# Rongjiehuang/FastDiff

Measured on AMD Instinct MI355X. Metric: real-time factor (audio-sec/wall-sec), N=4 reverse steps, 80x864 mel, higher is better.
Workload: dtype f32 results; 2-piece fp16 operands (22 bit) on fp16 MFMA, fp32 accumulate; GEMM as Winograd F(2,3); exact-fp32 twin; 1 GPU; BASELINE configs[1]: LJSpeech shape, batch=8 x 80x864 mel per GPU, N=4, HIP kernels + hipGraph sampler; batch_per_gpu=8, frames=864, reverse_steps=4, graph=True, weights=random init seed 1234 (no checkpoint offline), world_size=1, gpus_visible=1, oversubscribed=False

## Files before the change

fastdiff_amd/csrc/fd_api.cpp:

```cpp
#include <math.h>
#include <stddef.h>
#include <stdio.h>
#include <stdlib.h>
#include <string.h>

#include <algorithm>

#include "fd_kernels.h"
#include "fd_host.h"

std::string g_create_error;

static inline int gx_rows_host(int T) { return std::max(fdk_fast::gx_rows(T), fdk_fast::gw_pairs(T) * (fdk_fast::GW_ROWB / fdk_fast::GX_ROWB)); }

bool fd_prof_stamps(const fdk::Launch &L, const char *name, hipEvent_t *e0, hipEvent_t *e1)
{
    fd_context *c = L.ctx;
    if (c->profile != 1 || L.capturing) return false;
    hipEvent_t ev[2];
    for (int i = 0; i < 2; ++i) {
        if (!c->event_pool.empty()) { ev[i] = c->event_pool.back(); c->event_pool.pop_back(); }
        else if (hipEventCreate(&ev[i]) != hipSuccess) return false;
    }
    ProfEntry pe;
// ... 604 lines not shown
    h->pending.active = false;
    return resolve_call(h, p, mask);
}

static int sample_core(fd_handle h, const fd_context::SampleArgs &a, unsigned force_mask, long long ticket)
{
    int rc;
    const int B = a.B, T_io = a.T, T = bucket_frames(h, a.T), N = a.N;
    const int64_t L_io = (int64_t)T_io * fd::HOPT, Lp = (int64_t)T * fd::HOPT;
    hipStream_t stream = a.stream;
    Workspace &ws = h->ws;
    const size_t n_el = (size_t)B * T * fd::HOPT;
    const std::vector<unsigned long long> &ids = a.ids;
    constexpr int CHUNK = 8;
    StepMode mode = h->mode;
    const int np = hoist_mult(h, B, T, N);
    mode.hoist_np = np;
    mode.hoist_chunk = np > 1 && N > CHUNK;
    mode.fp32_mask = force_mask;
    mode.inline_fallback = force_mask != 0 || !h->host_fallback;
    std::vector<int> own_lens;
    const int *lens_eff = a.has_lens ? a.lens.data() : nullptr;
    if (!lens_eff && T != T_io) { own_lens.assign(B, T_io); lens_eff = own_lens.data(); }
    {
        fd_context::StageSlot *sl = nullptr;
        const size_t off_lens = sizeof(StepParams), off_ids = off_lens + ((sizeof(int) * B * np + 7) & ~(size_t)7);
        const size_t off_offs = off_ids + sizeof(unsigned long long) * B;
        const bool has_offs = !ids.empty() && !a.offs.empty();
        if ((rc = fd_stage_acquire(h, off_offs + sizeof(long long) * B, &sl)) != FD_OK) return rc;
        if ((rc = set_lens(h, lens_eff, B, T, stream, "fd_sample", reinterpret_cast<int *>(sl->host + off_lens), &mode.ragged, np)) != FD_OK)
            return rc;
        if (!ids.empty()) {
            memcpy(sl->host + off_ids, ids.data(), sizeof(unsigned long long) * B);
            FD_HIP(h, hipMemcpyAsync(ws.uid_dev, sl->host + off_ids, sizeof(unsigned long long) * B, hipMemcpyHostToDevice, stream));
        }
        if (has_offs) {
            memcpy(sl->host + off_offs, a.offs.data(), sizeof(long long) * B);
            FD_HIP(h, hipMemcpyAsync(ws.off_dev, sl->host + off_offs, sizeof(long long) * B, hipMemcpyHostToDevice, stream));
        }
        StepParams *p = reinterpret_cast<StepParams *>(sl->host);
        memcpy(p->table, a.table.data(), sizeof(fd_step) * N);
        p->z = a.z; p->seq = a.seq_out; p->seed = a.seed; p->n_steps = N; p->ddim = a.ddim ? 1 : 0; p->step_idx = 0; p->l4 = T * (fd::HOPT / 4);
        p->uids = ids.empty() ? nullptr : ws.uid_dev;
        p->offs4 = has_offs ? ws.off_dev : nullptr;
        p->l4_io = T_io * (fd::HOPT / 4); p->n4_io = (long long)B * p->l4_io;
        const size_t head = sizeof(fd_step) * N;
        FD_HIP(h, hipMemcpyAsync(ws.params, p, head, hipMemcpyHostToDevice, stream));
        const size_t off = offsetof(StepParams, z);
        FD_HIP(h, hipMemcpyAsync(reinterpret_cast<char *>(ws.params) + off, reinterpret_cast<const char *>(p) + off, sizeof(StepParams) - off,
                                 hipMemcpyHostToDevice, stream));
        if ((rc = fd_stage_commit(h, sl, stream)) != FD_OK) return rc;
    }
    fdk::Launch L = {h, stream, false, &mode};
    hipError_t e = fdk::copy_rows(L, ws.mel, T, a.mel, T_io, T_io, B * fd::COND);
    if (e == hipSuccess && a.x_T) e = fdk::copy_rows(L, ws.x, Lp, a.x_T, L_io, (int)L_io, B);
    if (e != hipSuccess) FD_FAIL(h, FD_ERR_HIP, "fd_sample: input copy failed: %s", hipGetErrorString(e));
    if (!a.x_T && (e = fdk::init_noise(L, ws.x, B, T * (fd::HOPT / 4), T_io * (fd::HOPT / 4), a.seed, ids.empty() ? nullptr : ws.uid_dev,
                                       ids.empty() || a.offs.empty() ? nullptr : ws.off_dev)) != hipSuccess)
        FD_FAIL(h, FD_ERR_HIP, "fd_sample: init_noise failed: %s", hipGetErrorString(e));
    if (a.seq_out && (e = fdk::copy_rows(L, a.seq_out, L_io, ws.x, Lp, (int)L_io, B)) != hipSuccess)
        FD_FAIL(h, FD_ERR_HIP, "fd_sample: sequence copy failed: %s", hipGetErrorString(e));
    auto copy_out = [&]() -> int {
        const hipError_t eo = fdk::copy_rows(L, a.out, L_io, ws.x, Lp, (int)L_io, B);
        if (eo != hipSuccess) FD_FAIL(h, FD_ERR_HIP, "fd_sample: output copy failed: %s", hipGetErrorString(eo));
        return FD_OK;
    };

    StepIO io = {ws.x, ws.mel, nullptr, nullptr, 1};
    {
        std::vector<float> ts(N);
        for (int k = 0; k < N; ++k) ts[k] = a.table[k].t;
        if (!(h->embed_cache && h->embed_valid && h->embed_B == B && h->embed_t == ts)) {
            h->embed_valid = false;
            if ((e = fdk::embed(L, io, B, N)) != hipSuccess) FD_FAIL(h, FD_ERR_HIP, "fd_sample: embed failed: %s", hipGetErrorString(e));
            h->embed_t.swap(ts);
            h->embed_B = B;
            h->embed_valid = true;
        }
    }
    if ((e = fdk::clear_range_flags(L)) != hipSuccess) FD_FAIL(h, FD_ERR_HIP, "fd_sample: %s", hipGetErrorString(e));

    if (np > 1) {
        const int64_t mel_n = (int64_t)B * fd::COND * T;
        if ((e = fdk::copy_rows(L, ws.mel_rep, T, ws.mel, T, T, B * fd::COND, np, mel_n)) != hipSuccess)
            FD_FAIL(h, FD_ERR_HIP, "fd_sample: mel replication failed: %s", hipGetErrorString(e));
    }
    if (np > 1 && !mode.hoist_chunk) {
        StepIO iop = {ws.x, ws.mel_rep, nullptr, nullptr, 0};
        e = fdk::kp_front(L, iop, B * N, T);
        if (e == hipSuccess) e = fdk::kp_gemm(L, B * N, T);
        if (e != hipSuccess) FD_FAIL(h, FD_ERR_HIP, "fd_sample: predictor launch failed: %s", hipGetErrorString(e));
    }
    if (force_mask != 0) {
        if ((rc = enqueue_steps(h, B, T, N, mode, stream)) != FD_OK) return rc;
        if ((rc = copy_out()) != FD_OK) return rc;
    } else if (h->host_fallback && N <= CHUNK) {
        if ((rc = enqueue_steps(h, B, T, N, mode, stream)) != FD_OK) return rc;
        const int slot = (int)(ticket & 1);
        FD_HIP(h, hipMemcpyAsync(h->flags_host + 32 * slot, ws.range_flag + 64, sizeof(int) * 32, hipMemcpyDeviceToHost, stream));
        FD_HIP(h, hipEventRecord(slot ? h->flags_done2 : h->flags_done, stream));
        if ((rc = copy_out()) != FD_OK) return rc;
        h->pending.active = true; h->pending.lazy = true; h->pending.slot = slot; h->pending.ticket = ticket;
        h->pending.B = B; h->pending.T = T; h->pending.T_io = T_io; h->pending.N = N; h->pending.first = 0; h->pending.count = N; h->pending.out = a.out;
        h->pending.stream = stream; h->pending.args = a;
    } else if (h->host_fallback) {
        FD_HIP(h, hipMemcpyAsync(ws.xsave, ws.x, sizeof(float) * n_el, hipMemcpyDeviceToDevice, stream));
        unsigned mask = 0;
        for (int first = 0; first < N; first += CHUNK) {
            const int count = std::min(CHUNK, N - first);
            const bool last = first + count == N;
            ++h->n_pieces;
            if (mask != 0) ++h->n_pieces_fp32;
            if (first > 0 && mask == 0) FD_HIP(h, hipMemcpyAsync(ws.xsave, ws.x, sizeof(float) * n_el, hipMemcpyDeviceToDevice, stream));
            mode.fp32_mask = mask;
            mode.inline_fallback = mask != 0;
            if ((rc = enqueue_steps(h, B, T, count, mode, stream)) != FD_OK) return rc;
            if (mask != 0) continue;
            FD_HIP(h, hipMemcpyAsync(h->flags_host, ws.range_flag + 64, sizeof(int) * 32, hipMemcpyDeviceToHost, stream));
            FD_HIP(h, hipEventRecord(h->flags_done, stream));
            h->pending.active = true; h->pending.lazy = false; h->pending.slot = 0; h->pending.ticket = ticket;
            h->pending.B = B; h->pending.T = T; h->pending.T_io = T_io; h->pending.N = N; h->pending.first = first; h->pending.count = count; h->pending.out = a.out;
            h->pending.stream = stream; h->pending.mode = mode;
            if (last) break;
            int redone = resolve_pending(h, &mask);
            if (redone < 0) return redone;
        }
        if ((rc = copy_out()) != FD_OK) return rc;
    } else {
        if ((rc = enqueue_steps(h, B, T, N, mode, stream)) != FD_OK) return rc;
        if ((rc = copy_out()) != FD_OK) return rc;
    }
    h->last_B = B; h->last_T = T;
    return fd_mark_tail(h, stream);
}

int fd_sample(fd_handle h, const float *mel, int B, int T, const int *lens, const fd_step *table, int N, int ddim,
              const float *x_T, const float *z, uint64_t seed, float *out, float *seq_out, void *stream_)
{
    std::vector<unsigned long long> ids;
    std::vector<long long> offs;
    if (h) { ids.swap(h->noise_ids); offs.swap(h->noise_offs); }
    int rc = check_common(h, B, T, "fd_sample");
    if (rc != FD_OK) return rc;
    if ((rc = fd_follow_stream(h, (hipStream_t)stream_)) != FD_OK) return rc;
    if (h->gen) {
        if (!mel || !table || !out) FD_FAIL(h, FD_ERR_INVALID, "fd_sample: null pointer");
        if (N <= 0 || N > 1024) FD_FAIL(h, FD_ERR_INVALID, "fd_sample: N=%d outside 1..1024", N);
        if (!ids.empty() && (int)ids.size() != B) FD_FAIL(h, FD_ERR_INVALID, "fd_sample: fd_set_noise_streams gave %d stream ids but B=%d", (int)ids.size(), B);
        for (int b = 0; lens && b < B; ++b)
            if (lens[b] < 1 || lens[b] > T) FD_FAIL(h, FD_ERR_INVALID, "fd_sample: lens[%d] = %d outside [1, T=%d]", b, lens[b], T);
        if ((rc = fdg::sample(h, mel, B, T, lens, table, N, ddim, x_T, z, seed, ids, out, seq_out, (hipStream_t)stream_)) != FD_OK) return rc;
        ++h->ticket_counter;
        h->last_B = B; h->last_T = T;
        return fd_mark_tail(h, (hipStream_t)stream_);
    }
    const bool lazy = h->host_fallback && N >= 1 && N <= 8;
    const int Tp = bucket_frames(h, T);
    if ((rc = check_common(h, B, Tp, "fd_sample")) != FD_OK) return rc;
    const int np = (N >= 1 && N <= 1024) ? hoist_mult(h, B, Tp, N) : 1;
    const bool ws_ok = workspace_fits(h, B, Tp, np);
    fd_context::PendingCall prev;
    if (lazy && ws_ok && h->pending.active && h->pending.lazy) {
        prev = h->pending;
        h->pending.active = false;
    } else if ((rc = fd_settle(h)) != FD_OK) return rc;
    auto finish_prev = [&]() -> int {
        if (!prev.active) return FD_OK;
        unsigned mask = 0;
        const fd_context::PendingCall cur = h->pending;
        h->pending.active = false;
        const int r = resolve_call(h, prev, &mask);
        h->pending = cur;
        prev.active = false;
        return r < 0 ? r : FD_OK;
    };
    if (!mel || !table || !out) { finish_prev(); FD_FAIL(h, FD_ERR_INVALID, "fd_sample: null pointer"); }
    if (N <= 0 || N > 1024) { finish_prev(); FD_FAIL(h, FD_ERR_INVALID, "fd_sample: N=%d outside 1..1024", N); }
    if (!ids.empty() && (int)ids.size() != B) {
        finish_prev();
        FD_FAIL(h, FD_ERR_INVALID, "fd_sample: fd_set_noise_streams gave %d stream ids but B=%d", (int)ids.size(), B);
    }
    if (!offs.empty() && offs.size() != ids.size()) { finish_prev(); FD_FAIL(h, FD_ERR_INVALID, "fd_sample: noise offsets without their stream ids"); }
    for (int b = 0; lens && b < B; ++b)
        if (lens[b] < 1 || lens[b] > T) {
            finish_prev();
            FD_FAIL(h, FD_ERR_INVALID, "fd_sample: lens[%d] = %d outside [1, T=%d]", b, lens[b], T);
        }
    if ((rc = ensure_workspace(h, B, Tp, np)) != FD_OK) { finish_prev(); return rc; }
    fd_context::SampleArgs a;
    a.mel = mel; a.B = B; a.T = T; a.N = N; a.ddim = ddim;
    a.has_lens = lens != nullptr;
    if (lens) a.lens.assign(lens, lens + B);
    a.table.assign(table, table + N);
    a.x_T = x_T; a.z = z; a.seed = seed; a.out = out; a.seq_out = seq_out; a.stream = (hipStream_t)stream_;
    a.ids.swap(ids);
    a.offs.swap(offs);
    const long long ticket = ++h->ticket_counter;
    h->n_pieces = h->n_pieces_redone = h->n_pieces_fp32 = 0;
    h->call_fp32_mask = 0;
    rc = sample_core(h, a, 0u, ticket);
    const int rc_prev = finish_prev();
    h->last_B = B; h->last_T = Tp;
    if (rc != FD_OK || rc_prev != FD_OK) return rc != FD_OK ? rc : rc_prev;
    if (!h->defer_check) return fd_settle(h);
    return FD_OK;
}

int64_t fd_sample_ticket(fd_handle h) { return h ? (int64_t)h->ticket_counter : FD_ERR_INVALID; }

static int ticket_redone(fd_handle h, long long ticket)
{
    for (long long t : h->redone_ring)
        if (t == ticket && t != 0) return 1;
    return 0;
}

int fd_sample_settle(fd_handle h, int64_t ticket)
{
    if (!h) return FD_ERR_INVALID;
    if (ticket <= 0 || ticket > h->ticket_counter) FD_FAIL(h, FD_ERR_INVALID, "fd_sample_settle: unknown ticket %lld", (long long)ticket);
    if (h->pending.active && h->pending.ticket <= ticket) {
        FD_HIP(h, hipSetDevice(h->device));
        unsigned mask = 0;
        const int r = resolve_pending(h, &mask);
        if (r < 0) return r;
    }
    return ticket_redone(h, ticket);
}

int fd_sample_check(fd_handle h)
{
    if (!h) return FD_ERR_INVALID;
    if (!h->pending.active) return 0;
    FD_HIP(h, hipSetDevice(h->device));
    unsigned mask = 0;
    return resolve_pending(h, &mask);
}

int fd_set_noise_streams(fd_handle h, const uint64_t *stream_ids, int B)
{
    if (!h || B < 0 || (B > 0 && !stream_ids)) return FD_ERR_INVALID;
    h->noise_ids.assign(stream_ids, stream_ids + B);
    h->noise_offs.clear();
    return FD_OK;
}

int fd_set_option(fd_handle h, const char *key, const char *value)
{
    if (!h || !key || !value) return FD_ERR_INVALID;
    {
        const int rcs = fd_settle(h);
        if (rcs != FD_OK) return rcs;
    }
    const std::string k(key), v(value);
    static const char *stage_names[ST_COUNT] = {"embed", "first", "dblock", "kp_front", "kp_gemm", "convt", "lvc", "final"};
    auto parse_mode = [&](bool &dst) -> int {
        if (v == "fast") dst = true;
        else if (v == "naive") dst = false;
        else FD_FAIL(h, FD_ERR_INVALID, "fd_set_option: %s expects fast|naive, got '%s'", key, value);
        return FD_OK;
    };
    if (k == "kernels") {
        bool m = true;
        int rc = parse_mode(m);
        if (rc != FD_OK) return rc;
        for (int i = 0; i < ST_COUNT; ++i) h->mode.fast[i] = m;
        return FD_OK;
    }
    if (k.compare(0, 8, "kernels.") == 0) {
        for (int i = 0; i < ST_COUNT; ++i)
            if (k.substr(8) == stage_names[i]) return parse_mode(h->mode.fast[i]);
        FD_FAIL(h, FD_ERR_INVALID, "fd_set_option: unknown stage '%s'", key);
    }
    static const struct { const char *key, *a, *b; void (*set)(fd_context *, bool); } choices[] = {
        {"gemm", "f16x2", "fp32", [](fd_context *c, bool a) { c->mode.gemm_f16 = a; }},
        {"gemm_form", "winograd", "direct", [](fd_context *c, bool a) { c->mode.gemm_wino = a; }},
        {"lvc", "f16x2", "fp32", [](fd_context *c, bool a) { c->mode.lvc_f16 = a; }},
        {"conv", "f16x2", "fp32", [](fd_context *c, bool a) { c->mode.conv_f16 = a; }},
        {"lvc_h8", "mfma", "valu", [](fd_context *c, bool a) { c->mode.lvc_h8_mfma = a; }},
        {"fallback", "graph", "host", [](fd_context *c, bool a) { c->host_fallback = !a; }},
        {"lvc_dx", "gather", "copy", [](fd_context *c, bool a) { c->lvc_dx_gather = a; }},
        {"mel", "pwg", "tacotron", [](fd_context *c, bool a) { c->mel_variant = a ? MEL_PWG : MEL_TACOTRON; }},
    };
    for (const auto &ch : choices) {
        if (k != ch.key) continue;
        if (v != ch.a && v != ch.b) FD_FAIL(h, FD_ERR_INVALID, "fd_set_option: %s expects %s|%s, got '%s'", key, ch.a, ch.b, value);
        ch.set(h, v == ch.a);
        return FD_OK;
    }
    const bool on = (v == "1" || v == "true" || v == "on");
    if (k == "fuse_final") { h->mode.fuse_final = on; return FD_OK; }
    if (k == "fuse_up") { h->mode.fuse_up = on; return FD_OK; }
    if (k == "fuse_advance") { h->mode.fuse_advance = on; return FD_OK; }
    if (k == "embed_cache") { h->embed_cache = on; return FD_OK; }
    if (k == "hoist") {
        if (v == "auto") h->hoist_mode = 1;
        else if (v == "on") h->hoist_mode = 2;
        else if (v == "off") h->hoist_mode = 0;
        else FD_FAIL(h, FD_ERR_INVALID, "fd_set_option: hoist expects auto|on|off, got '%s'", value);
        return FD_OK;
    }
    if (k == "graph") { h->use_graph = on; return FD_OK; }
    if (k == "defer_check") { h->defer_check = on; return FD_OK; }
    if (k == "t_bucket" || k == "graph_cache") {
        char *end = nullptr;
        const long n = strtol(value, &end, 10);
        if (end == value || *end != 0 || n < 0 || n > 65536 || (k == "graph_cache" && n < 1))
            FD_FAIL(h, FD_ERR_INVALID, "fd_set_option: %s expects an integer (t_bucket: frames, 0 = exact T; graph_cache: graphs kept, >= 1), got '%s'", key, value);
        if (k == "t_bucket") h->t_bucket = (int)n;
        else h->max_graphs = (int)n;
        return FD_OK;
    }
    if (k == "profile") { h->profile = (v == "events") ? 2 : (on ? 1 : 0); return FD_OK; }
    if (k == "taps") { h->mode.keep_taps = on; return FD_OK; }
    FD_FAIL(h, FD_ERR_INVALID, "fd_set_option: unknown option '%s'", key);
}

}
```

fastdiff_amd/csrc/fd_internal.h:

```cpp
#pragma once
#include <hip/hip_runtime.h>
#include <hip/hip_ext.h>
#include <stdint.h>
#include <string.h>
#include <map>
#include <string>
#include <vector>

#include "../../include/fastdiff_hip.h"
#include "../../include/fastdiff_hip_ext.h"
#include "../../include/fastdiff_hip_train.h"

namespace fd {
constexpr int C = 32;
constexpr int COND = 80;
constexpr int HID = 64;
constexpr int NBLK = 3;
constexpr int LAYERS = 4;
constexpr int HOPT = 256;
constexpr int E_IN = 128, E_MID = 512, E_OUT = 512;
constexpr int KLAYER = 2 * C * C * 3;
constexpr int KW = KLAYER * LAYERS;
constexpr int KB = 2 * C * LAYERS;
constexpr int KREC = KW + KB;
__host__ __device__ constexpr int ratio(int n) { return n == 2 ? 4 : 8; }
__host__ __device__ constexpr int hop(int n) { return n == 0 ? 8 : (n == 1 ? 64 : 256); }
__host__ __device__ constexpr int down_factor(int d) { return d == 0 ? 4 : 8; }

__host__ __device__ inline int kernel_row(int out) { return (out & 15) + 16 * (out >> 5); }
__host__ __device__ inline int kernel_tile(int out) { return (out & 31) >> 4; }
__host__ __device__ inline int kernel_index(int layer, int in, int out, int tap)
{
    const int kk = tap * C + in, kg = kk >> 4, g = (kk >> 3) & 1, e = kk & 7;
    const int mt = kernel_tile(out), lane = kernel_row(out) + 32 * g;
    return layer * KLAYER + ((mt * 6 + kg) * 64 + lane) * 8 + e;
}
__host__ __device__ inline int bias_index(int layer, int out) { return KW + layer * 64 + kernel_tile(out) * 32 + kernel_row(out); }
}

struct ConvW {
    const float *w = nullptr;
    const float *b = nullptr;
};

struct DevWeights {
    ConvW first, final_;
    struct { ConvW res, conv[3]; } down[fd::NBLK];
    struct { ConvW fc_t, up, kp_in, kp_res[6], kc, bc, convs[fd::LAYERS]; } blk[fd::NBLK];
    const float *fc_t1_T = nullptr, *fc_t1_b = nullptr, *fc_t2_T = nullptr, *fc_t2_b = nullptr;
    const float *fc_t_T[fd::NBLK] = {}, *fc_t_b[fd::NBLK] = {};
    const float *embed_table = nullptr;
    const float *down_pack[fd::NBLK][4] = {};
    const uint16_t *down_h2[fd::NBLK][4] = {};
    bool dblock_f16_ok = false;
    const float *lvc_conv_pack[fd::NBLK][fd::LAYERS] = {};
    const uint16_t *lvc_conv_h2[fd::NBLK][fd::LAYERS] = {};
    const uint16_t *lvc_conv_h16[fd::LAYERS] = {};
    bool lvc_f16_ok = false;
    const float *kp_in_pack[fd::NBLK] = {};
    const float *kp_res_pack[fd::NBLK][6] = {};
    const uint16_t *kp_in_h2[fd::NBLK] = {};
    const uint16_t *kp_res_h2[fd::NBLK][6] = {};
    bool kpf_f16_ok = false;
    const float *gemm_pack[fd::NBLK] = {};
    const float *gemm_bias[fd::NBLK] = {};
    const uint16_t *gemm_h2_pack[fd::NBLK] = {};
    bool gemm_f16_ok = false;
    const uint16_t *gemm_w_pack[fd::NBLK] = {};
    bool gemm_w_ok = false;
    const float *up_pack[fd::NBLK] = {};
    const uint16_t *up_h2[fd::NBLK] = {};
    bool convt_f16_ok = false;
    const float *final_fuse = nullptr;
    const int *kc_perm = nullptr;
    const int *bc_perm = nullptr;
};

struct StepParams {
    fd_step table[1024];
    const float *z;
    float *seq;
    unsigned long long seed;
    int n_steps;
    int ddim;
    int step_idx;
    int l4;
    const unsigned long long *uids;
    int l4_io;
    long long n4_io;
    const long long *offs4;
};

enum Stage { ST_EMBED = 0, ST_FIRST, ST_DBLOCK, ST_KP_FRONT, ST_KP_GEMM, ST_CONVT, ST_LVC, ST_FINAL, ST_COUNT };

struct StepMode {
    bool fast[ST_COUNT] = {true, true, true, true, true, true, true, true};
    bool gemm_f16 = true;
    bool gemm_wino = true;
    bool lvc_f16 = true;
    bool conv_f16 = true;
    bool lvc_h8_mfma = true;
    bool fuse_final = true;
    bool fuse_up = true;
    bool fuse_advance = true;
    bool keep_taps = false;
    unsigned fp32_mask = 0;
    bool inline_fallback = true;
    bool ragged = false;
    int hoist_np = 1;
    bool hoist_chunk = false;

    bool operator==(const StepMode &o) const
    {
        for (int i = 0; i < ST_COUNT; ++i)
            if (fast[i] != o.fast[i]) return false;
        return gemm_f16 == o.gemm_f16 && gemm_wino == o.gemm_wino && lvc_f16 == o.lvc_f16 && conv_f16 == o.conv_f16 &&
               lvc_h8_mfma == o.lvc_h8_mfma && fuse_final == o.fuse_final && fuse_up == o.fuse_up && fuse_advance == o.fuse_advance &&
               keep_taps == o.keep_taps && fp32_mask == o.fp32_mask && inline_fallback == o.inline_fallback && ragged == o.ragged &&
               hoist_np == o.hoist_np && hoist_chunk == o.hoist_chunk;
    }
};

struct Workspace {
    int B = 0;
    int64_t frames = 0;
    int64_t rows = 0;
    float *noise = nullptr;
    float *embed_h2 = nullptr;
    float *a[4] = {};
    float *kp_h0 = nullptr, *kp_hA = nullptr, *kp_hB = nullptr;
    float *kpack = nullptr;
    float *h_f16 = nullptr;
    int *lens_dev = nullptr;
    unsigned long long *uid_dev = nullptr;
    long long *off_dev = nullptr;
    float *xsave = nullptr;
    int *range_flag = nullptr;
    float *xA = nullptr, *xB = nullptr;
    float *xtap[fd::NBLK] = {};
    int64_t pframes = 0, prows = 0, plens = 0;
    float *mel_rep = nullptr;
    float *mel = nullptr;
    float *x = nullptr;
    float *eps_acc = nullptr;
    float *steps = nullptr;
    StepParams *params = nullptr;
    size_t bytes = 0;
};

struct ProfEntry { std::string name; hipEvent_t e0, e1; };
struct Scratch { float *p = nullptr; size_t bytes = 0; };

struct MelTables {
    const float *tab = nullptr;
    const int *fb_lo = nullptr, *fb_n = nullptr, *fb_off = nullptr;
    const float *fb_w = nullptr;
};
enum MelVariant { MEL_PWG = 0, MEL_TACOTRON = 1, MEL_VARIANTS = 2 };

struct FoldedParam { std::vector<float> w, b; };
struct WeightImage {
    std::vector<char> bytes;
    std::vector<std::pair<const void **, size_t>> fields;
    template <class T> void add(const T *&dst, const std::vector<T> &v)
    {
        const size_t off = (bytes.size() + 255) & ~(size_t)255;
        bytes.resize(off + v.size() * sizeof(T));
        memcpy(bytes.data() + off, v.data(), v.size() * sizeof(T));
        fields.push_back({reinterpret_cast<const void **>(&dst), off});
    }
};
namespace fdg {
struct Net;
int validate(const fd_config &c, std::string &why);
int create(fd_context *c);
void destroy(fd_context *c);
int hop_total(const fd_context *c);
int pack_weights(fd_context *c, const std::map<std::string, FoldedParam> &f, WeightImage &img);
int forward(fd_context *c, const float *x, const float *mel, const float *steps, int B, int T, const int *lens, float *eps_out, hipStream_t stream);
int sample(fd_context *c, const float *mel, int B, int T, const int *lens, const fd_step *table, int N, int ddim, const float *x_T, const float *z,
           unsigned long long seed, const std::vector<unsigned long long> &ids, float *out, float *seq_out, hipStream_t stream);
}

struct fd_context {
    fd_config cfg;
    fdg::Net *gen = nullptr;
    int device = 0;
    int num_cus = 256;
    std::string err;
    bool committed = false;
    StepMode mode;
    bool use_graph = true;
    int profile = 0;
    std::vector<unsigned long long> noise_ids;
    std::vector<long long> noise_offs;
    bool host_fallback = true;
    std::map<std::string, std::pair<std::vector<int64_t>, std::vector<float>>> raw;
    void *weight_arena = nullptr;
    DevWeights w;
    Workspace ws;
    bool lvc_dx_gather = true;
    std::vector<float> embed_t;
    int embed_B = 0;
    bool embed_valid = false;
    bool embed_cache = true;
    MelTables mel[MEL_VARIANTS];
    int mel_variant = MEL_PWG;
    std::vector<float> mel_bank[MEL_VARIANTS];
    bool mel_bank_user[MEL_VARIANTS] = {false, false};
    std::vector<void *> mel_allocs;
    int last_B = 0, last_T = 0;
    hipStream_t cap_stream = nullptr;
    hipStream_t last_stream = nullptr;
    bool have_last_stream = false;
    hipEvent_t ev_switch = nullptr;
    bool tail_marked = false;
    int hoist_mode = 1;
    struct StepGraph { int B, T, steps; StepMode mode; hipGraph_t graph; hipGraphExec_t exec; unsigned long long last_use; };
    std::vector<StepGraph> graphs;
    unsigned long long graph_clock = 0;
    struct RetiredGraph { hipGraph_t graph; hipGraphExec_t exec; hipEvent_t done; };
    std::vector<RetiredGraph> retired;
    int max_graphs = 64;
    int t_bucket = 32;
    long long n_graph_captures = 0, n_graph_hits = 0, n_graph_evictions = 0;
    bool defer_check = false;
    static constexpr int STAGE_SLOTS = 8;
    struct StageSlot { char *host = nullptr; size_t cap = 0; hipEvent_t done = nullptr; };
    StageSlot stage[STAGE_SLOTS];
    unsigned stage_next = 0;
    struct SampleArgs {
        const float *mel = nullptr;
        int B = 0, T = 0, N = 0, ddim = 0;
        bool has_lens = false;
        std::vector<int> lens;
        std::vector<fd_step> table;
        const float *x_T = nullptr, *z = nullptr;
        unsigned long long seed = 0;
        float *out = nullptr, *seq_out = nullptr;
        hipStream_t stream = nullptr;
        std::vector<unsigned long long> ids;
        std::vector<long long> offs;
    };
    struct PendingCall {
        bool active = false;
        bool lazy = false;
        int slot = 0;
        long long ticket = 0;
        int B = 0, T = 0, N = 0, first = 0, count = 0;
        int T_io = 0;
        float *out = nullptr;
        hipStream_t stream = nullptr;
        StepMode mode;
        SampleArgs args;
    } pending;
    long long ticket_counter = 0;
    long long n_pieces = 0, n_pieces_redone = 0, n_pieces_fp32 = 0, n_calls_redone = 0;
    unsigned call_fp32_mask = 0;
    long long redone_ring[16] = {};
    unsigned redone_next = 0;
    int *flags_host = nullptr;
    hipEvent_t flags_done = nullptr, flags_done2 = nullptr;
    void *scratch = nullptr;
    Scratch lvc_scratch;
    Scratch kconv_scratch;
    Scratch cconv_scratch;
    Scratch span_scratch;
    Scratch step_scratch;
    std::vector<ProfEntry> prof_pending;
    std::vector<hipEvent_t> event_pool;
    std::map<std::string, std::pair<int64_t, double>> prof_acc;
};

enum Pipe { PIPE_F16_THEN_F32, PIPE_F16_ONLY, PIPE_F32_ONLY };
inline Pipe fd_pipe(const StepMode &m, bool f16_possible, int flag_word)
{
    if (!f16_possible || ((m.fp32_mask >> flag_word) & 1u)) return PIPE_F32_ONLY;
    return m.inline_fallback ? PIPE_F16_THEN_F32 : PIPE_F16_ONLY;
}
inline bool front_writes_h_image(const StepMode &m, const DevWeights &w)
{
    return m.fast[ST_KP_FRONT] && fd_pipe(m, m.conv_f16 && w.kpf_f16_ok, 19) != PIPE_F32_ONLY &&
           fd_pipe(m, m.gemm_f16 && w.gemm_f16_ok, 0) != PIPE_F32_ONLY && !(m.gemm_wino && w.gemm_w_ok);
}
inline bool last_lvc_fuses_final(const StepMode &m, const DevWeights &w)
{
    return m.fast[ST_LVC] && m.fast[ST_FINAL] && !m.keep_taps && m.fuse_final &&
           fd_pipe(m, m.lvc_f16 && w.lvc_f16_ok, 1 + 2 * fd::LAYERS + 3) != PIPE_F32_ONLY;
}

struct StepIO {
    const float *x_in;
    const float *mel;
    const float *steps;
    float *eps_out;
    int sampler;
    int hoist_step = 0;
    bool advance = false;
};

namespace fdk {
struct Launch {
    fd_context *ctx;
    hipStream_t stream;
    bool capturing;
    const StepMode *mode = nullptr;
};
hipError_t embed(const Launch &L, const StepIO &io, int B, int n_steps);
hipError_t first_conv(const Launch &L, const StepIO &io, int B, int T);
hipError_t dblock(const Launch &L, const StepIO &io, int d, int B, int T);
hipError_t kp_front(const Launch &L, const StepIO &io, int B, int T);
hipError_t kp_gemm(const Launch &L, int B, int T);
hipError_t advance_step(const Launch &L);
hipError_t clear_range_flags(const Launch &L, int set_step = 0);
hipError_t mel_frontend(const Launch &L, const float *wav, int B, int64_t n_samples, float *mel, int T);
hipError_t init_noise(const Launch &L, float *x, int B, int l4, int l4_io, unsigned long long seed, const unsigned long long *uids,
                      const long long *offs4 = nullptr);
constexpr int SPAN_MAX_WINDOWS = 8;
struct SpanWindows {
    int n;
    long long start[SPAN_MAX_WINDOWS];
    int len[SPAN_MAX_WINDOWS];
    long long c0[SPAN_MAX_WINDOWS];
    int clen[SPAN_MAX_WINDOWS];
};
hipError_t span_gather(const Launch &L, const SpanWindows &w, int Wp, const float *mel, const float *x_T, const float *z, int nz,
                       long long mel_first, long long mel_frames, float *mel_w, float *x_w, float *z_w);
hipError_t span_scatter(const Launch &L, const SpanWindows &w, int Wp, const float *x_w, long long t0, float *out);
hipError_t copy_rows(const Launch &L, float *dst, int64_t dpitch, const float *src, int64_t spitch, int width, int rows, int reps = 1,
                     int64_t rep_stride = 0);
hipError_t peak_normalize_int16(const Launch &L, const float *wav, int B, int64_t len, int16_t *pcm, const long long *valid_dev);
}

bool fd_prof_stamps(const fdk::Launch &L, const char *name, hipEvent_t *e0, hipEvent_t *e1);
void fd_prof_begin(const fdk::Launch &L, const char *name);
void fd_prof_end(const fdk::Launch &L);

#define FD_LAUNCH(L, name, kernel, grid, block, shmem, ...)                                  \
    do {                                                                                     \
        hipEvent_t ev0__ = nullptr, ev1__ = nullptr;                                         \
        if (fd_prof_stamps(L, name, &ev0__, &ev1__)) {                                       \
            hipExtLaunchKernelGGL(kernel, grid, block, shmem, (L).stream, ev0__, ev1__, 0, __VA_ARGS__); \
        } else {                                                                             \
            fd_prof_begin(L, name);                                                          \
            hipLaunchKernelGGL(kernel, grid, block, shmem, (L).stream, __VA_ARGS__);         \
            fd_prof_end(L);                                                                  \
        }                                                                                    \
        hipError_t e__ = hipGetLastError();                                                  \
        if (e__ != hipSuccess) return e__;                                                   \
    } while (0)
```

fastdiff_amd/csrc/fd_kernels_dblock.hip:

```cpp
#include "fd_kernels_common.h"

namespace fdk_fast {

constexpr int DB_LD = 136;
constexpr int DB_STRIDE = 114;

template <int DIL, bool LRELU>
__device__ __forceinline__ void conv96_tile(f32x16 &acc, const float4 (&wa)[12], const float *in, int ld, int col, int hi)
{
    const int o[3] = {opaque(hi * ld + col - DIL), opaque(hi * ld + col), opaque(hi * ld + col + DIL)};
#pragma unroll
    for (int s = 0; s < 48; ++s) {
        const int tap = s >> 4, c2 = (2 * s) & 31;
        float v = in[o[tap] + c2 * ld];
        if (LRELU) v = lrelu(v, 0.2f);
        acc = mfma32(f4c(wa[s >> 2], s & 3), v, acc);
    }
}

template <int F>
__global__ void __launch_bounds__(256, 2) k_dblock(const float *__restrict__ xin, float *__restrict__ out,
                                                   const float *__restrict__ p0, const float *__restrict__ p1,
                                                   const float *__restrict__ p2, const float *__restrict__ pr,
                                                   const float *__restrict__ b0, const float *__restrict__ b1,
                                                   const float *__restrict__ b2, const float *__restrict__ br, int Lin, int Lo,
                                                   const int *__restrict__ run_if, const int *__restrict__ lens, int per_frame)
{
    __shared__ __attribute__((aligned(16))) float xs[fd::C * DB_LD];
    if (run_if && *run_if == 0) return;
    __shared__ __attribute__((aligned(16))) float hA[fd::C * DB_LD];
    __shared__ __attribute__((aligned(16))) float hB[fd::C * DB_LD];
    const int b = blockIdx.y, tid = threadIdx.x, lane = tid & 63, wave = tid >> 6, l31 = lane & 31, hi = lane >> 5;
    const int pbase = blockIdx.x * DB_STRIDE - 7;
    const int Lob = lens ? lens[b] * per_frame : Lo;
    if (blockIdx.x * DB_STRIDE >= Lob) return;
    {
        constexpr int NK = fd::C * DB_LD / 256;
        float v[NK];
#pragma unroll
        for (int k = 0; k < NK; ++k) {
            const int idx = k * 256 + tid, ci = idx / DB_LD, cc = idx - ci * DB_LD, p = pbase + cc - 4;
            v[k] = (cc >= 4 && cc < 132 && p >= 0 && p < Lob) ? xin[((int64_t)b * fd::C + ci) * Lin + (int64_t)p * F] : 0.0f;
        }
#pragma unroll
        for (int k = 0; k < NK; ++k) {
            const int idx = k * 256 + tid;
            xs[idx] = v[k];
            hA[idx] = 0.0f;
            hB[idx] = 0.0f;
        }
    }
    __syncthreads();
    const int c = wave * 32 + l31;
    const int p = pbase + c;
    const bool inside = (p >= 0 && p < Lob);
    float4 wa[12];
    f32x16 acc;
#pragma unroll
    for (int i = 0; i < 12; ++i) wa[i] = reinterpret_cast<const float4 *>(p0)[i * 64 + lane];
#pragma unroll
    for (int r = 0; r < 16; ++r) acc[r] = b0[drow(r, hi)];
    conv96_tile<1, true>(acc, wa, xs, DB_LD, 4 + c, hi);
#pragma unroll
    for (int r = 0; r < 16; ++r) hA[drow(r, hi) * DB_LD + 4 + c] = inside ? acc[r] : 0.0f;
    __syncthreads();
#pragma unroll
    for (int i = 0; i < 12; ++i) wa[i] = reinterpret_cast<const float4 *>(p1)[i * 64 + lane];
#pragma unroll
    for (int r = 0; r < 16; ++r) acc[r] = b1[drow(r, hi)];
    conv96_tile<2, true>(acc, wa, hA, DB_LD, 4 + c, hi);
#pragma unroll
    for (int r = 0; r < 16; ++r) hB[drow(r, hi) * DB_LD + 4 + c] = inside ? acc[r] : 0.0f;
    __syncthreads();
#pragma unroll
    for (int i = 0; i < 12; ++i) wa[i] = reinterpret_cast<const float4 *>(p2)[i * 64 + lane];
#pragma unroll
    for (int r = 0; r < 16; ++r) acc[r] = b2[drow(r, hi)] + br[drow(r, hi)];
    conv96_tile<4, true>(acc, wa, hB, DB_LD, 4 + c, hi);
    {
        float4 wr[4];
#pragma unroll
        for (int i = 0; i < 4; ++i) wr[i] = reinterpret_cast<const float4 *>(pr)[i * 64 + lane];
#pragma unroll
        for (int s = 0; s < 16; ++s) acc = mfma32(f4c(wr[s >> 2], s & 3), xs[(2 * s + hi) * DB_LD + 4 + c], acc);
    }
    if (inside && c >= 7 && c < 7 + DB_STRIDE) {
#pragma unroll
        for (int r = 0; r < 16; ++r) out[((int64_t)b * fd::C + drow(r, hi)) * Lo + p] = acc[r];
    }
}

constexpr int DBH_ROWS = 136;

template <int DIL>
__device__ __forceinline__ void conv96_h2(f32x16 &ah, f32x16 &al, const float4 (&wa)[2][6], const char *img, int c, int hi)
{
    int off[3][2][2];
#pragma unroll
    for (int tap = 0; tap < 3; ++tap)
#pragma unroll
        for (int p = 0; p < 2; ++p)
#pragma unroll
            for (int c2 = 0; c2 < 2; ++c2) off[tap][p][c2] = h2_off(4 + c + (tap - 1) * DIL, p * 4 + c2 * 2 + hi);
#pragma unroll
    for (int kg = 0; kg < 6; ++kg) {
        const float4 b1 = *reinterpret_cast<const float4 *>(img + off[kg >> 1][0][kg & 1]);
        const float4 b2 = *reinterpret_cast<const float4 *>(img + off[kg >> 1][1][kg & 1]);
        ah = mfma_f16(wa[0][kg], b1, ah);
        al = mfma_f16(wa[0][kg], b2, al);
        al = mfma_f16(wa[1][kg], b1, al);
    }
}
__device__ __forceinline__ void store_act_h2(char *img, const f32x16 &ah, const f32x16 &al, int c, int hi, bool inside, float &mx)
{
    const int row = 4 + c;
#pragma unroll
    for (int j = 0; j < 4; ++j) {
        float v[4];
#pragma unroll
        for (int i = 0; i < 4; ++i) {
            v[i] = inside ? lrelu(fmaf(al[4 * j + i], GX_INV_SCALE, ah[4 * j + i]), 0.2f) : 0.0f;
            mx = fmaxf(mx, fabsf(v[i]));
        }
        uint2 ph, pl;
        split2(v[0], v[1], ph.x, pl.x);
        split2(v[2], v[3], ph.y, pl.y);
        *reinterpret_cast<uint2 *>(img + h2_off(row, j) + 8 * hi) = ph;
        *reinterpret_cast<uint2 *>(img + h2_off(row, 4 + j) + 8 * hi) = pl;
    }
}

#ifndef FD_DBLOCK_OCC
#define FD_DBLOCK_OCC 3
#endif
template <int F, bool AUDIO>
__global__ void __launch_bounds__(256, FD_DBLOCK_OCC) k_dblock_h2(const float *__restrict__ xin, float *__restrict__ out,
                                                      const float4 *__restrict__ p0, const float4 *__restrict__ p1,
                                                      const float4 *__restrict__ p2, const float4 *__restrict__ pr,
                                                      const float *__restrict__ b0, const float *__restrict__ b1,
                                                      const float *__restrict__ b2, const float *__restrict__ br, int Lin, int Lo,
                                                      int *__restrict__ range_flag, const int *__restrict__ lens, int per_frame,
                                                      const float *__restrict__ audio, const float *__restrict__ fw,
                                                      const float *__restrict__ fb)
{
    __shared__ __attribute__((aligned(16))) char xl[DBH_ROWS * 128];
    __shared__ __attribute__((aligned(16))) char xr[DBH_ROWS * 128];
    __shared__ __attribute__((aligned(16))) char ha[DBH_ROWS * 128];
    const int b = blockIdx.y, tid = threadIdx.x, lane = tid & 63, wave = tid >> 6, l31 = lane & 31, hi = lane >> 5;
    const int pbase = blockIdx.x * DB_STRIDE - 7;
    const int Lob = lens ? lens[b] * per_frame : Lo;
    if (blockIdx.x * DB_STRIDE >= Lob || skip_after_previous_overflow(range_flag)) return;
    float mx = 0.0f;
    __shared__ float fwl[AUDIO ? 256 : 1];
    if constexpr (AUDIO) {
        fwl[tid] = tid < 224 ? fw[tid] : fb[tid - 224];
        __syncthreads();
    }
    {
        float v[2][8];
#pragma unroll
        for (int k = 0; k < 2; ++k) {
            const int u = k * 256 + tid, cg = u >> 7, cc = u & 127, p = pbase + cc;
            const bool ok = p >= 0 && p < Lob;
            if (AUDIO) {
                const int Lb = Lob * F, t = p * F;
                const float *xa = audio + (int64_t)b * Lin;
                float xv[7];
#pragma unroll
                for (int i = 0; i < 7; ++i) xv[i] = (ok && t - 3 + i >= 0 && t - 3 + i < Lb) ? xa[t - 3 + i] : 0.0f;
                const int o0 = __builtin_amdgcn_readfirstlane(cg) * 8;
#pragma unroll
                for (int c = 0; c < 8; ++c) {
                    float r = fwl[224 + o0 + c];
#pragma unroll
                    for (int i = 0; i < 7; ++i) r += fwl[(o0 + c) * 7 + i] * xv[i];
                    v[k][c] = ok ? r : 0.0f;
                }
            } else {
#pragma unroll
                for (int c = 0; c < 8; ++c) v[k][c] = ok ? xin[((int64_t)b * fd::C + cg * 8 + c) * Lin + (int64_t)p * F] : 0.0f;
            }
        }
        if (tid < 128) {
            const int g = tid >> 4, row = g < 4 ? g : 128 + g, part = tid & 15;
            *reinterpret_cast<uint2 *>(xl + row * 128 + part * 8) = make_uint2(0u, 0u);
            *reinterpret_cast<uint2 *>(xr + row * 128 + part * 8) = make_uint2(0u, 0u);
            *reinterpret_cast<uint2 *>(ha + row * 128 + part * 8) = make_uint2(0u, 0u);
        }
#pragma unroll
        for (int k = 0; k < 2; ++k) {
            const int u = k * 256 + tid, cg = u >> 7, cc = u & 127;
            float a[8];
#pragma unroll
            for (int c = 0; c < 8; ++c) { mx = fmaxf(mx, fabsf(v[k][c])); a[c] = lrelu(v[k][c], 0.2f); }
            float4 ph, pl;
            split8(v[k], ph, pl);
            *reinterpret_cast<float4 *>(xr + h2_off(4 + cc, cg)) = ph;
            *reinterpret_cast<float4 *>(xr + h2_off(4 + cc, 4 + cg)) = pl;
            split8(a, ph, pl);
            *reinterpret_cast<float4 *>(xl + h2_off(4 + cc, cg)) = ph;
            *reinterpret_cast<float4 *>(xl + h2_off(4 + cc, 4 + cg)) = pl;
        }
    }
    __syncthreads();
    const int c = wave * 32 + l31;
    const int p = pbase + c;
    const bool inside = (p >= 0 && p < Lob);
    float4 wa[2][6];
    f32x16 ah, al;
    auto load_w = [&](const float4 *pk) {
#pragma unroll
        for (int q = 0; q < 2; ++q)
#pragma unroll
            for (int kg = 0; kg < 6; ++kg) wa[q][kg] = pk[(q * 6 + kg) * 64 + lane];
    };
    load_w(p0);
#pragma unroll
    for (int r = 0; r < 16; ++r) { ah[r] = b0[drow(r, hi)]; al[r] = 0.0f; }
    conv96_h2<1>(ah, al, wa, xl, c, hi);
    store_act_h2(ha, ah, al, c, hi, inside, mx);
    __syncthreads();
    load_w(p1);
#pragma unroll
    for (int r = 0; r < 16; ++r) { ah[r] = b1[drow(r, hi)]; al[r] = 0.0f; }
    conv96_h2<2>(ah, al, wa, ha, c, hi);
    store_act_h2(xl, ah, al, c, hi, inside, mx);
    __syncthreads();
    load_w(p2);
#pragma unroll
    for (int r = 0; r < 16; ++r) { ah[r] = b2[drow(r, hi)] + br[drow(r, hi)]; al[r] = 0.0f; }
    conv96_h2<4>(ah, al, wa, xl, c, hi);
    {
        float4 wr[2][2];
#pragma unroll
        for (int q = 0; q < 2; ++q)
#pragma unroll
            for (int kg = 0; kg < 2; ++kg) wr[q][kg] = pr[(q * 2 + kg) * 64 + lane];
#pragma unroll
        for (int kg = 0; kg < 2; ++kg) {
            const float4 x1 = *reinterpret_cast<const float4 *>(xr + h2_off(4 + c, kg * 2 + hi));
            const float4 x2 = *reinterpret_cast<const float4 *>(xr + h2_off(4 + c, 4 + kg * 2 + hi));
            ah = mfma_f16(wr[0][kg], x1, ah);
            al = mfma_f16(wr[0][kg], x2, al);
            al = mfma_f16(wr[1][kg], x1, al);
        }
    }
    if (inside && c >= 7 && c < 7 + DB_STRIDE) {
#pragma unroll
        for (int r = 0; r < 16; ++r) out[((int64_t)b * fd::C + drow(r, hi)) * Lo + p] = fmaf(al[r], GX_INV_SCALE, ah[r]);
    }
    if (!(mx < GX_LIMIT)) atomicOr(range_flag, 1);
}

}

namespace fdk {
using namespace fdk_fast;

hipError_t fast_dblock(const Launch &L, int d, int B, int T, const float *audio)
{
    fd_context *c = L.ctx;
    const DevWeights &w = c->w;
    int Lin = T * fd::HOPT;
    for (int i = 0; i < d; ++i) Lin /= fd::down_factor(i);
    const int f = fd::down_factor(d), Lo = Lin / f;
    const dim3 grid((Lo + DB_STRIDE - 1) / DB_STRIDE, B);
    const int *run_if = nullptr;
    const char *n4 = "dblock_f4", *n8 = "dblock_f8";
    const int *lens = L.mode->ragged ? c->ws.lens_dev : nullptr;
    const Pipe pipe = fd_pipe(*L.mode, L.mode->conv_f16 && w.dblock_f16_ok, 13 + d);
    if (pipe != PIPE_F32_ONLY) {
        int *flag = c->ws.range_flag + 13 + d;
        const float4 *q0 = reinterpret_cast<const float4 *>(w.down_h2[d][0]), *q1 = reinterpret_cast<const float4 *>(w.down_h2[d][1]),
                     *q2 = reinterpret_cast<const float4 *>(w.down_h2[d][2]), *q3 = reinterpret_cast<const float4 *>(w.down_h2[d][3]);
        const float *none = nullptr;
        if (f == 4 && d == 0 && audio)
            FD_LAUNCH(L, n4, (k_dblock_h2<4, true>), grid, dim3(256), 0, c->ws.a[d], c->ws.a[d + 1], q0, q1, q2, q3, w.down[d].conv[0].b,
                      w.down[d].conv[1].b, w.down[d].conv[2].b, w.down[d].res.b, Lin, Lo, flag, lens, Lo / T, audio,
                      (const float *)w.first.w, (const float *)w.first.b);
        else if (f == 4)
            FD_LAUNCH(L, n4, (k_dblock_h2<4, false>), grid, dim3(256), 0, c->ws.a[d], c->ws.a[d + 1], q0, q1, q2, q3, w.down[d].conv[0].b,
                      w.down[d].conv[1].b, w.down[d].conv[2].b, w.down[d].res.b, Lin, Lo, flag, lens, Lo / T, none, none, none);
        else
            FD_LAUNCH(L, n8, (k_dblock_h2<8, false>), grid, dim3(256), 0, c->ws.a[d], c->ws.a[d + 1], q0, q1, q2, q3, w.down[d].conv[0].b,
                      w.down[d].conv[1].b, w.down[d].conv[2].b, w.down[d].res.b, Lin, Lo, flag, lens, Lo / T, none, none, none);
        run_if = flag;
        n4 = n8 = "dblock_fp32_fallback";
        if (pipe == PIPE_F16_ONLY) return hipSuccess;
    }
    if (f == 4)
        FD_LAUNCH(L, n4, k_dblock<4>, grid, dim3(256), 0, c->ws.a[d], c->ws.a[d + 1], w.down_pack[d][0], w.down_pack[d][1],
                  w.down_pack[d][2], w.down_pack[d][3], w.down[d].conv[0].b, w.down[d].conv[1].b, w.down[d].conv[2].b,
                  w.down[d].res.b, Lin, Lo, run_if, lens, Lo / T);
    else
        FD_LAUNCH(L, n8, k_dblock<8>, grid, dim3(256), 0, c->ws.a[d], c->ws.a[d + 1], w.down_pack[d][0], w.down_pack[d][1],
                  w.down_pack[d][2], w.down_pack[d][3], w.down[d].conv[0].b, w.down[d].conv[1].b, w.down[d].conv[2].b,
                  w.down[d].res.b, Lin, Lo, run_if, lens, Lo / T);
    return hipSuccess;
}

}
```

Baseline: 10030 x real-time.

## Make fp16 downsampling block persistent with register-resident weights and prefetch

Turns the split-fp16 dblock kernel into a persistent kernel. A capped grid (two workgroups per CU by default, or set by a new dblock_wgs option) loops over tiles. All three conv weight sets stay in registers, and biases plus residual weights move to LDS once per workgroup. The next tile's global input is fetched during the last conv of the current tile, and the conv inner loop double-buffers its LDS operand loads behind sched barriers. This removes the per-tile weight reload and launch tail, at the cost of higher register pressure, which is why occupancy drops from 3 to 2, and adds an extra barrier per tile.

```diff
diff --git a/fastdiff_amd/csrc/fd_api.cpp b/fastdiff_amd/csrc/fd_api.cpp
--- a/fastdiff_amd/csrc/fd_api.cpp
+++ b/fastdiff_amd/csrc/fd_api.cpp
@@ -930,6 +930,19 @@
     }
     if (k == "graph") { h->use_graph = on; return FD_OK; }
     if (k == "defer_check") { h->defer_check = on; return FD_OK; }
+    if (k == "dblock_wgs") {
+        char *end = nullptr;
+        const long n = strtol(value, &end, 10);
+        if (end == value || *end != 0 || n < 0 || n > 65536)
+            FD_FAIL(h, FD_ERR_INVALID, "fd_set_option: dblock_wgs expects an integer (workgroups, 0 = two per CU), got '%s'", value);
+        if ((int)n != h->dblock_wgs) {
+            FD_HIP(h, hipSetDevice(h->device));
+            FD_HIP(h, hipDeviceSynchronize());
+            drop_graph(h);
+        }
+        h->dblock_wgs = (int)n;
+        return FD_OK;
+    }
     if (k == "t_bucket" || k == "graph_cache") {
         char *end = nullptr;
         const long n = strtol(value, &end, 10);
diff --git a/fastdiff_amd/csrc/fd_internal.h b/fastdiff_amd/csrc/fd_internal.h
--- a/fastdiff_amd/csrc/fd_internal.h
+++ b/fastdiff_amd/csrc/fd_internal.h
@@ -187,6 +187,7 @@
     fdg::Net *gen = nullptr;
     int device = 0;
     int num_cus = 256;
+    int dblock_wgs = 0;
     std::string err;
     bool committed = false;
     StepMode mode;
diff --git a/fastdiff_amd/csrc/fd_kernels_dblock.hip b/fastdiff_amd/csrc/fd_kernels_dblock.hip
--- a/fastdiff_amd/csrc/fd_kernels_dblock.hip
+++ b/fastdiff_amd/csrc/fd_kernels_dblock.hip
@@ -95,20 +95,20 @@
 template <int DIL>
 __device__ __forceinline__ void conv96_h2(f32x16 &ah, f32x16 &al, const float4 (&wa)[2][6], const char *img, int c, int hi)
 {
-    int off[3][2][2];
-#pragma unroll
-    for (int tap = 0; tap < 3; ++tap)
-#pragma unroll
-        for (int p = 0; p < 2; ++p)
-#pragma unroll
-            for (int c2 = 0; c2 < 2; ++c2) off[tap][p][c2] = h2_off(4 + c + (tap - 1) * DIL, p * 4 + c2 * 2 + hi);
+    auto ld = [&](int kg, int p) { return *reinterpret_cast<const float4 *>(img + h2_off(4 + c + ((kg >> 1) - 1) * DIL, p * 4 + (kg & 1) * 2 + hi)); };
+    float4 b1[2], b2[2];
+    b1[0] = ld(0, 0);
+    b2[0] = ld(0, 1);
 #pragma unroll
     for (int kg = 0; kg < 6; ++kg) {
-        const float4 b1 = *reinterpret_cast<const float4 *>(img + off[kg >> 1][0][kg & 1]);
-        const float4 b2 = *reinterpret_cast<const float4 *>(img + off[kg >> 1][1][kg & 1]);
-        ah = mfma_f16(wa[0][kg], b1, ah);
-        al = mfma_f16(wa[0][kg], b2, al);
-        al = mfma_f16(wa[1][kg], b1, al);
+        if (kg < 5) {
+            b1[(kg + 1) & 1] = ld(kg + 1, 0);
+            b2[(kg + 1) & 1] = ld(kg + 1, 1);
+        }
+        ah = mfma_f16(wa[0][kg], b1[kg & 1], ah);
+        al = mfma_f16(wa[0][kg], b2[kg & 1], al);
+        al = mfma_f16(wa[1][kg], b1[kg & 1], al);
+        __builtin_amdgcn_sched_barrier(0);
     }
 }
 __device__ __forceinline__ void store_act_h2(char *img, const f32x16 &ah, const f32x16 &al, int c, int hi, bool inside, float &mx)
@@ -131,7 +131,7 @@
 }
 
 #ifndef FD_DBLOCK_OCC
-#define FD_DBLOCK_OCC 3
+#define FD_DBLOCK_OCC 2
 #endif
 template <int F, bool AUDIO>
 __global__ void __launch_bounds__(256, FD_DBLOCK_OCC) k_dblock_h2(const float *__restrict__ xin, float *__restrict__ out,
@@ -141,113 +141,153 @@
                                                       const float *__restrict__ b2, const float *__restrict__ br, int Lin, int Lo,
                                                       int *__restrict__ range_flag, const int *__restrict__ lens, int per_frame,
                                                       const float *__restrict__ audio, const float *__restrict__ fw,
-                                                      const float *__restrict__ fb)
+                                                      const float *__restrict__ fb, int tiles_x, int ntiles)
 {
     __shared__ __attribute__((aligned(16))) char xl[DBH_ROWS * 128];
     __shared__ __attribute__((aligned(16))) char xr[DBH_ROWS * 128];
     __shared__ __attribute__((aligned(16))) char ha[DBH_ROWS * 128];
-    const int b = blockIdx.y, tid = threadIdx.x, lane = tid & 63, wave = tid >> 6, l31 = lane & 31, hi = lane >> 5;
-    const int pbase = blockIdx.x * DB_STRIDE - 7;
-    const int Lob = lens ? lens[b] * per_frame : Lo;
-    if (blockIdx.x * DB_STRIDE >= Lob || skip_after_previous_overflow(range_flag)) return;
+    __shared__ float fwl[AUDIO ? 256 : 1];
+    __shared__ float4 wrl[2][2][64];
+    __shared__ __attribute__((aligned(16))) float bl[96];
+    const int tid = threadIdx.x, lane = tid & 63, wave = tid >> 6, l31 = lane & 31, hi = lane >> 5;
+    float4 w0[2][6], w1[2][6], w2[2][6];
+#pragma unroll
+    for (int q = 0; q < 2; ++q)
+#pragma unroll
+        for (int kg = 0; kg < 6; ++kg) {
+            w0[q][kg] = p0[(q * 6 + kg) * 64 + lane];
+            w1[q][kg] = p1[(q * 6 + kg) * 64 + lane];
+            w2[q][kg] = p2[(q * 6 + kg) * 64 + lane];
+        }
+    const float4 wv = pr[tid];
+    float bv = 0.0f, fv = 0.0f;
+    if (tid < 96) bv = tid < 32 ? b0[tid] : (tid < 64 ? b1[tid - 32] : b2[tid - 64] + br[tid - 64]);
+    if constexpr (AUDIO) fv = tid < 224 ? fw[tid] : fb[tid - 224];
+    if (skip_after_previous_overflow(range_flag)) return;
+
+    constexpr int NG = AUDIO ? 7 : 8;
+    struct Tile { int b, pbase, Lob; };
+    auto next_tile = [&](int n, Tile &t) {
+        for (; n < ntiles; n += gridDim.x) {
+            t.b = n / tiles_x;
+            t.pbase = (n - t.b * tiles_x) * DB_STRIDE - 7;
+            t.Lob = lens ? lens[t.b] * per_frame : Lo;
+            if (t.pbase + 7 < t.Lob) break;
+        }
+        return n;
+    };
+    auto fetch = [&](float (&g)[2][NG], const Tile &t) {
+        const int tf = opaque(tid);
+#pragma unroll
+        for (int k = 0; k < 2; ++k) {
+            const int u = k * 256 + tf, cg = u >> 7, cc = u & 127, p = t.pbase + cc;
+            const bool ok = p >= 0 && p < t.Lob;
+            if constexpr (AUDIO) {
+                const int Lb = t.Lob * F, s = p * F;
+                const float *xa = audio + (int64_t)t.b * Lin;
+#pragma unroll
+                for (int i = 0; i < 7; ++i) g[k][i] = (ok && s - 3 + i >= 0 && s - 3 + i < Lb) ? xa[s - 3 + i] : 0.0f;
+            } else {
+#pragma unroll
+                for (int c = 0; c < 8; ++c) g[k][c] = ok ? xin[((int64_t)t.b * fd::C + cg * 8 + c) * Lin + (int64_t)p * F] : 0.0f;
+            }
+        }
+    };
+
+    Tile cur, nxt;
+    int n = next_tile(blockIdx.x, cur);
+    if (n >= ntiles) return;
+    float g[2][NG];
+    fetch(g, cur);
+    if constexpr (AUDIO) fwl[tid] = fv;
+    if (tid < 96) bl[tid] = bv;
+    (&wrl[0][0][0])[tid] = wv;
+    if (tid < 128) {
+        const int gq = tid >> 4, row = gq < 4 ? gq : 128 + gq, part = tid & 15;
+        *reinterpret_cast<uint2 *>(xl + row * 128 + part * 8) = make_uint2(0u, 0u);
+        *reinterpret_cast<uint2 *>(xr + row * 128 + part * 8) = make_uint2(0u, 0u);
+        *reinterpret_cast<uint2 *>(ha + row * 128 + part * 8) = make_uint2(0u, 0u);
+    }
+    if constexpr (AUDIO) __syncthreads();
     float mx = 0.0f;
-    __shared__ float fwl[AUDIO ? 256 : 1];
-    if constexpr (AUDIO) {
-        fwl[tid] = tid < 224 ? fw[tid] : fb[tid - 224];
-        __syncthreads();
-    }
-    {
-        float v[2][8];
+    const int c0 = wave * 32 + l31;
+    f32x16 ah, al;
+    auto start = [&](int layer) {
+#pragma unroll
+        for (int j = 0; j < 4; ++j) {
+            const float4 t = *reinterpret_cast<const float4 *>(bl + layer * 32 + 8 * j + 4 * hi);
+            ah[4 * j] = t.x; ah[4 * j + 1] = t.y; ah[4 * j + 2] = t.z; ah[4 * j + 3] = t.w;
+        }
+#pragma unroll
+        for (int r = 0; r < 16; ++r) al[r] = 0.0f;
+    };
+    for (;;) {
+        const int ts = opaque(tid);
 #pragma unroll
         for (int k = 0; k < 2; ++k) {
-            const int u = k * 256 + tid, cg = u >> 7, cc = u & 127, p = pbase + cc;
-            const bool ok = p >= 0 && p < Lob;
-            if (AUDIO) {
-                const int Lb = Lob * F, t = p * F;
-                const float *xa = audio + (int64_t)b * Lin;
-                float xv[7];
-#pragma unroll
-                for (int i = 0; i < 7; ++i) xv[i] = (ok && t - 3 + i >= 0 && t - 3 + i < Lb) ? xa[t - 3 + i] : 0.0f;
+            const int u = k * 256 + ts, cg = u >> 7, cc = u & 127, p = cur.pbase + cc;
+            const bool ok = p >= 0 && p < cur.Lob;
+            float v[8];
+            if constexpr (AUDIO) {
                 const int o0 = __builtin_amdgcn_readfirstlane(cg) * 8;
 #pragma unroll
-                for (int c = 0; c < 8; ++c) {
-                    float r = fwl[224 + o0 + c];
-#pragma unroll
-                    for (int i = 0; i < 7; ++i) r += fwl[(o0 + c) * 7 + i] * xv[i];
-                    v[k][c] = ok ? r : 0.0f;
+                for (int ch = 0; ch < 8; ++ch) {
+                    float r = fwl[224 + o0 + ch];
+#pragma unroll
+                    for (int i = 0; i < 7; ++i) r += fwl[(o0 + ch) * 7 + i] * g[k][i];
+                    v[ch] = ok ? r : 0.0f;
                 }
             } else {
 #pragma unroll
-                for (int c = 0; c < 8; ++c) v[k][c] = ok ? xin[((int64_t)b * fd::C + cg * 8 + c) * Lin + (int64_t)p * F] : 0.0f;
+                for (int ch = 0; ch < 8; ++ch) v[ch] = g[k][ch];
             }
-        }
-        if (tid < 128) {
-            const int g = tid >> 4, row = g < 4 ? g : 128 + g, part = tid & 15;
-            *reinterpret_cast<uint2 *>(xl + row * 128 + part * 8) = make_uint2(0u, 0u);
-            *reinterpret_cast<uint2 *>(xr + row * 128 + part * 8) = make_uint2(0u, 0u);
-            *reinterpret_cast<uint2 *>(ha + row * 128 + part * 8) = make_uint2(0u, 0u);
-        }
-#pragma unroll
-        for (int k = 0; k < 2; ++k) {
-            const int u = k * 256 + tid, cg = u >> 7, cc = u & 127;
             float a[8];
 #pragma unroll
-            for (int c = 0; c < 8; ++c) { mx = fmaxf(mx, fabsf(v[k][c])); a[c] = lrelu(v[k][c], 0.2f); }
+            for (int ch = 0; ch < 8; ++ch) { mx = fmaxf(mx, fabsf(v[ch])); a[ch] = lrelu(v[ch], 0.2f); }
             float4 ph, pl;
-            split8(v[k], ph, pl);
+            split8(v, ph, pl);
             *reinterpret_cast<float4 *>(xr + h2_off(4 + cc, cg)) = ph;
             *reinterpret_cast<float4 *>(xr + h2_off(4 + cc, 4 + cg)) = pl;
             split8(a, ph, pl);
             *reinterpret_cast<float4 *>(xl + h2_off(4 + cc, cg)) = ph;
             *reinterpret_cast<float4 *>(xl + h2_off(4 + cc, 4 + cg)) = pl;
         }
-    }
-    __syncthreads();
-    const int c = wave * 32 + l31;
-    const int p = pbase + c;
-    const bool inside = (p >= 0 && p < Lob);
-    float4 wa[2][6];
-    f32x16 ah, al;
-    auto load_w = [&](const float4 *pk) {
-#pragma unroll
-        for (int q = 0; q < 2; ++q)
-#pragma unroll
-            for (int kg = 0; kg < 6; ++kg) wa[q][kg] = pk[(q * 6 + kg) * 64 + lane];
-    };
-    load_w(p0);
-#pragma unroll
-    for (int r = 0; r < 16; ++r) { ah[r] = b0[drow(r, hi)]; al[r] = 0.0f; }
-    conv96_h2<1>(ah, al, wa, xl, c, hi);
-    store_act_h2(ha, ah, al, c, hi, inside, mx);
-    __syncthreads();
-    load_w(p1);
-#pragma unroll
-    for (int r = 0; r < 16; ++r) { ah[r] = b1[drow(r, hi)]; al[r] = 0.0f; }
-    conv96_h2<2>(ah, al, wa, ha, c, hi);
-    store_act_h2(xl, ah, al, c, hi, inside, mx);
-    __syncthreads();
-    load_w(p2);
-#pragma unroll
-    for (int r = 0; r < 16; ++r) { ah[r] = b2[drow(r, hi)] + br[drow(r, hi)]; al[r] = 0.0f; }
-    conv96_h2<4>(ah, al, wa, xl, c, hi);
-    {
-        float4 wr[2][2];
-#pragma unroll
-        for (int q = 0; q < 2; ++q)
-#pragma unroll
-            for (int kg = 0; kg < 2; ++kg) wr[q][kg] = pr[(q * 2 + kg) * 64 + lane];
+        __syncthreads();
+        const int p = cur.pbase + c0;
+        const bool inside = (p >= 0 && p < cur.Lob);
+        int c = opaque(c0);
+        start(0);
+        conv96_h2<1>(ah, al, w0, xl, c, hi);
+        store_act_h2(ha, ah, al, c, hi, inside, mx);
+        __syncthreads();
+        c = opaque(c0);
+        start(1);
+        conv96_h2<2>(ah, al, w1, ha, c, hi);
+        store_act_h2(xl, ah, al, c, hi, inside, mx);
+        __syncthreads();
+        n = next_tile(n + gridDim.x, nxt);
+        const bool more = n < ntiles;
+        if (more) fetch(g, nxt);
+        c = opaque(c0);
+        start(2);
+        conv96_h2<4>(ah, al, w2, xl, c, hi);
 #pragma unroll
         for (int kg = 0; kg < 2; ++kg) {
             const float4 x1 = *reinterpret_cast<const float4 *>(xr + h2_off(4 + c, kg * 2 + hi));
             const float4 x2 = *reinterpret_cast<const float4 *>(xr + h2_off(4 + c, 4 + kg * 2 + hi));
-            ah = mfma_f16(wr[0][kg], x1, ah);
-            al = mfma_f16(wr[0][kg], x2, al);
-            al = mfma_f16(wr[1][kg], x1, al);
-        }
-    }
-    if (inside && c >= 7 && c < 7 + DB_STRIDE) {
-#pragma unroll
-        for (int r = 0; r < 16; ++r) out[((int64_t)b * fd::C + drow(r, hi)) * Lo + p] = fmaf(al[r], GX_INV_SCALE, ah[r]);
+            const float4 r1 = wrl[0][kg][lane], r2 = wrl[1][kg][lane];
+            ah = mfma_f16(r1, x1, ah);
+            al = mfma_f16(r1, x2, al);
+            al = mfma_f16(r2, x1, al);
+        }
+        if (inside && c >= 7 && c < 7 + DB_STRIDE) {
+            const int ho = opaque(hi);
+#pragma unroll
+            for (int r = 0; r < 16; ++r) out[((int64_t)cur.b * fd::C + drow(r, ho)) * Lo + p] = fmaf(al[r], GX_INV_SCALE, ah[r]);
+        }
+        if (!more) break;
+        cur = nxt;
+        __syncthreads();
     }
     if (!(mx < GX_LIMIT)) atomicOr(range_flag, 1);
 }
@@ -270,20 +310,22 @@
     const int *lens = L.mode->ragged ? c->ws.lens_dev : nullptr;
     const Pipe pipe = fd_pipe(*L.mode, L.mode->conv_f16 && w.dblock_f16_ok, 13 + d);
     if (pipe != PIPE_F32_ONLY) {
+        const int tiles_x = (int)grid.x, ntiles = tiles_x * B, slots = c->dblock_wgs > 0 ? c->dblock_wgs : FD_DBLOCK_OCC * c->num_cus;
+        const dim3 pgrid(ntiles < slots ? ntiles : slots);
         int *flag = c->ws.range_flag + 13 + d;
         const float4 *q0 = reinterpret_cast<const float4 *>(w.down_h2[d][0]), *q1 = reinterpret_cast<const float4 *>(w.down_h2[d][1]),
                      *q2 = reinterpret_cast<const float4 *>(w.down_h2[d][2]), *q3 = reinterpret_cast<const float4 *>(w.down_h2[d][3]);
         const float *none = nullptr;
         if (f == 4 && d == 0 && audio)
-            FD_LAUNCH(L, n4, (k_dblock_h2<4, true>), grid, dim3(256), 0, c->ws.a[d], c->ws.a[d + 1], q0, q1, q2, q3, w.down[d].conv[0].b,
+            FD_LAUNCH(L, n4, (k_dblock_h2<4, true>), pgrid, dim3(256), 0, c->ws.a[d], c->ws.a[d + 1], q0, q1, q2, q3, w.down[d].conv[0].b,
                       w.down[d].conv[1].b, w.down[d].conv[2].b, w.down[d].res.b, Lin, Lo, flag, lens, Lo / T, audio,
-                      (const float *)w.first.w, (const float *)w.first.b);
+                      (const float *)w.first.w, (const float *)w.first.b, tiles_x, ntiles);
         else if (f == 4)
-            FD_LAUNCH(L, n4, (k_dblock_h2<4, false>), grid, dim3(256), 0, c->ws.a[d], c->ws.a[d + 1], q0, q1, q2, q3, w.down[d].conv[0].b,
-                      w.down[d].conv[1].b, w.down[d].conv[2].b, w.down[d].res.b, Lin, Lo, flag, lens, Lo / T, none, none, none);
+            FD_LAUNCH(L, n4, (k_dblock_h2<4, false>), pgrid, dim3(256), 0, c->ws.a[d], c->ws.a[d + 1], q0, q1, q2, q3, w.down[d].conv[0].b,
+                      w.down[d].conv[1].b, w.down[d].conv[2].b, w.down[d].res.b, Lin, Lo, flag, lens, Lo / T, none, none, none, tiles_x, ntiles);
         else
-            FD_LAUNCH(L, n8, (k_dblock_h2<8, false>), grid, dim3(256), 0, c->ws.a[d], c->ws.a[d + 1], q0, q1, q2, q3, w.down[d].conv[0].b,
-                      w.down[d].conv[1].b, w.down[d].conv[2].b, w.down[d].res.b, Lin, Lo, flag, lens, Lo / T, none, none, none);
+            FD_LAUNCH(L, n8, (k_dblock_h2<8, false>), pgrid, dim3(256), 0, c->ws.a[d], c->ws.a[d + 1], q0, q1, q2, q3, w.down[d].conv[0].b,
+                      w.down[d].conv[1].b, w.down[d].conv[2].b, w.down[d].res.b, Lin, Lo, flag, lens, Lo / T, none, none, none, tiles_x, ntiles);
         run_if = flag;
         n4 = n8 = "dblock_fp32_fallback";
         if (pipe == PIPE_F16_ONLY) return hipSuccess;
```

After: 10060 x real-time, median of 6. Within noise of the previous version (+0.3%).
